# michiyasunaga/qagnn

Hardware: AMD Instinct MI355X
Metric: QA-subgraphs/sec (batch x num_choice) fwd+bwd (higher is better)
Workload: dtype f32; 1 GPU; configs[1]: CSQA-shaped batch 64 questions x 5 choices = 320 subgraphs per GPU, n=200 node slots, 400..2000 edges/subgraph, 38 relations (run_qagnn__csqa.sh), 5-layer GAT d=200 H=4, QAGNN decoder fwd+bwd (LM encoder excluded: random sent_vecs), dropout 0.2, train-mode BN; subgraphs_per_gpu=320, nodes=64000, edges=396800, edges_with_self_loops=460800, graph_input=load-time int32 blobs (qagnn_graph_from_blobs), 13.3 B/edge on the wire, parallelism=single

## Files before the change

qagnn_amd/csrc/gemm_nn2.hip:

```cpp
#include <stdlib.h>

#include <atomic>

#include "common.h"

namespace qagnn {


namespace nn2 {

#ifndef QAGNN_NN2_ABL
#define QAGNN_NN2_ABL 0
#endif

constexpr int BK = 32;
constexpr uint32_t OOB = 0x80000000u;

__device__ __forceinline__ u32x4s bload(__amdgpu_buffer_rsrc_t rsrc, uint32_t voff, uint32_t soff) {
  return __builtin_bit_cast(u32x4s, __builtin_amdgcn_raw_buffer_load_b128(rsrc, (int)voff, (int)soff, 0));
}

__device__ __forceinline__ void split3(uint32_t u, uint32_t& h1, uint32_t& h2, uint32_t& h3) {
  h1 = u & 0xFFFF0000u;
  const float r1 = __builtin_bit_cast(float, u) - __builtin_bit_cast(float, h1);
// ... 365 lines not shown
        }
        QAGNN_NN2_BAR
        QAGNN_NN2_MFMA_TILE3(cur)
        QAGNN_NN2_BAR_VM
      }
      if (g == 0) QAGNN_NN2_BAR
    } else {
    if constexpr (PACKED) {
      QAGNN_NN2_GLDS(0, smem)
    } else {
#pragma unroll
      for (int q = 0; q < BR; ++q) QAGNN_NN2_STORE_B(q, smem)
    }
    QAGNN_NN2_SPLIT_A(0)
    __syncthreads();
    for (int it = 0; it + 1 < nkt; ++it) {
      unsigned char* const cur = smem + (it & 1) * IMG;
      unsigned char* const nxt = smem + ((it & 1) ^ 1) * IMG;
      if constexpr (PACKED && !(QAGNN_NN2_ABL & 2)) QAGNN_NN2_GLDS(it + 1, nxt)
      if constexpr (!(QAGNN_NN2_ABL & 1)) QAGNN_NN2_GLOAD(it + 1)
      QAGNN_NN2_MFMA_TILE(cur, nxt, !PACKED && !(QAGNN_NN2_ABL & 2))
      if constexpr (!(QAGNN_NN2_ABL & 4)) QAGNN_NN2_SPLIT_A(it + 1)
      if constexpr (!(QAGNN_NN2_ABL & 8)) __syncthreads();
    }
    {
      unsigned char* const cur = smem + ((nkt - 1) & 1) * IMG;
      QAGNN_NN2_MFMA_TILE(cur, cur, false)
    }
    }
    if constexpr (NP <= 2) {
      const uint32_t* const bfield = reinterpret_cast<const uint32_t*>(pk + ((int64_t)nkt * ldn1 + 13) * (NP * 1024)) + n0 / 16;
#pragma unroll
      for (int j = 0; j < NT; ++j) {
        const float inv = h2_inv_scale(fa, bfield[j]);
#pragma unroll
        for (int i = 0; i < 2; ++i) acc[i][j] *= inv;
      }
    }
    if constexpr (DIRECT) {
      const int em0 = m0, en0 = n0;
      if constexpr (STAG) {
        loaded = vb + (int)gridDim.x < ntiles;
        if (loaded) {
          QAGNN_NN2_SET_TILE(vb + (int)gridDim.x)
          QAGNN_NN2_FIRST_LOADS
        }
      }
      const __amdgpu_buffer_rsrc_t rC = __builtin_amdgcn_make_buffer_rsrc(a.C, 0, M * a.ldc * 4, 0x00020000);
      const int c4 = 4 * (lane >> 4);
      uint32_t crow[2];
#pragma unroll
      for (int i = 0; i < 2; ++i) {
        const int row = em0 + w * 32 + i * 16 + (lane & 15);
        const bool rok = row < M;
        crow[i] = rok ? (uint32_t)row * (uint32_t)a.ldc * 4u : OOB;
        f32x4s t[NT];
        if (a.bias) {
#pragma unroll
          for (int j = 0; j < NT; ++j) t[j] = __builtin_bit_cast(f32x4s, ld4(a.bias + min(en0 + j * 16 + c4, No - 4)));
#pragma unroll
          for (int j = 0; j < NT; ++j) acc[i][j] += t[j];
        }
        if (a.rowtab) {
          const float* const trow = a.rowtab + (int64_t)a.rowidx[rok ? row : 0] * a.ldt;
#pragma unroll
          for (int j = 0; j < NT; ++j) t[j] = __builtin_bit_cast(f32x4s, ld4(trow + min(en0 + j * 16 + c4, No - 4)));
#pragma unroll
          for (int j = 0; j < NT; ++j) acc[i][j] += t[j];
        }
        if (a.accumulate) {
#pragma unroll
          for (int j = 0; j < NT; ++j) {
            const int col = en0 + j * 16 + c4;
            t[j] = __builtin_bit_cast(f32x4s, bload(rC, rok && col < No ? crow[i] + (uint32_t)col * 4u : OOB, 0u));
          }
#pragma unroll
          for (int j = 0; j < NT; ++j) acc[i][j] += t[j];
        }
      }
#pragma unroll
      for (int i = 0; i < 2; ++i)
#pragma unroll
        for (int j = 0; j < NT; ++j) {
          const int col = en0 + j * 16 + c4;
          const uint32_t off = crow[i] != OOB && col < No ? crow[i] + (uint32_t)col * 4u : OOB;
          if constexpr (QAGNN_NN2_ABL & 64) {
            if (acc[i][j][0] == 1.2345e-30f) __builtin_amdgcn_raw_buffer_store_b128(__builtin_bit_cast(u32x4s, acc[i][j]), rC, (int)off, 0, 0);
          } else {
            __builtin_amdgcn_raw_buffer_store_b128(__builtin_bit_cast(u32x4s, acc[i][j]), rC, (int)off, 0, 0);
          }
        }
      continue;
    }
#undef QAGNN_NN2_FRAG
#undef QAGNN_NN2_FRAG_WAIT
#undef QAGNN_NN2_MFMA_TILE3
#undef QAGNN_NN2_BAR
#undef QAGNN_NN2_BAR_VM
#undef QAGNN_NN2_BAR_VMN
#undef QAGNN_NN2_FIRST_LOADS
#undef QAGNN_NN2_GLOAD
#undef QAGNN_NN2_SET_TILE
#undef QAGNN_NN2_GLDS
#undef QAGNN_NN2_STORE_B
#undef QAGNN_NN2_SPLIT_A
#undef QAGNN_NN2_MFMA_TILE

    float* const St = reinterpret_cast<float*>(smem) + w * SLAB_ROWS * PS;
    float (*const cstat)[2][BN] = reinterpret_cast<float (*)[2][BN]>(smem + SLAB_B);
    constexpr int ROW_F4 = BN / 4, TILE_F4 = SLAB_ROWS * ROW_F4, ST_IT = (TILE_F4 + 63) / 64;
    constexpr int SC = (BN + 63) / 64;
    float x0r[SC], s1[SC], s2v[SC];
#pragma unroll
    for (int cc = 0; cc < SC; ++cc) x0r[cc] = s1[cc] = s2v[cc] = 0.f;
#pragma unroll
    for (int i = 0; i < 2; ++i) {
      __syncthreads();
      const int lr0 = (lane >> 4) * 4;
#pragma unroll
      for (int j = 0; j < NT; ++j)
#pragma unroll
        for (int r = 0; r < 4; ++r) St[(lr0 + r) * PS + j * 16 + (lane & 15)] = acc[i][j][r];
      __syncthreads();
      if constexpr (STATS) {
        const float* const S0 = reinterpret_cast<const float*>(smem) + (w & ~3) * SLAB_ROWS * PS;
#pragma unroll
        for (int cc = 0; cc < SC; ++cc) {
          const int c = lane + cc * 64;
          if (c < BN && n0 + c < No) {
            const float bcv = a.bias ? a.bias[n0 + c] : 0.f;
            if (i == 0) x0r[cc] = S0[c] + bcv;
            const int rows = M - (m0 + (w * 2 + i) * 16);
            float v[SLAB_ROWS];
#pragma unroll
            for (int r = 0; r < SLAB_ROWS; ++r) v[r] = St[r * PS + c];
#pragma unroll
            for (int r = 0; r < SLAB_ROWS; ++r) {
              const float dlt = r < rows ? (v[r] + bcv) - x0r[cc] : 0.f;
              s1[cc] += dlt;
              s2v[cc] = fmaf(dlt, dlt, s2v[cc]);
            }
          }
        }
      }
#pragma unroll
      for (int itx = 0; itx < ST_IT; ++itx) {
        const int idx = lane + itx * 64;
        if (idx >= TILE_F4) break;
        const int slr = idx / ROW_F4, c4 = idx % ROW_F4;
        const int row = m0 + (w * 2 + i) * 16 + slr, col = n0 + c4 * 4;
        if (row >= M || col >= No) continue;
        float4 v = ld4(St + slr * PS + c4 * 4);
        if (a.bias) v = add4(v, ld4(a.bias + col));
        if (a.rowtab) v = add4(v, ld4(a.rowtab + (int64_t)a.rowidx[row] * a.ldt + col));
        float* dst = a.C + (int64_t)row * a.ldc + col;
        if (a.accumulate) v = add4(v, ld4(dst));
        if constexpr (QAGNN_NN2_ABL & 64) {
          if (v.x == 1.2345e-30f) st4(dst, v);
        } else {
          st4(dst, v);
        }
      }
    }
    if constexpr (STATS) {
#pragma unroll
      for (int cc = 0; cc < SC; ++cc) {
        const int c = lane + cc * 64;
        if (c < BN) { cstat[w][0][c] = s1[cc]; cstat[w][1][c] = s2v[cc]; }
      }
      __syncthreads();
      const int hw = w & 3, hf = w >> 2, col = hw * 64 + lane;
      if (col < BN && n0 + col < No && m0 + hf * 128 < M) {
        float x0c = x0r[0];
#pragma unroll
        for (int cc = 1; cc < SC; ++cc) x0c = (hw == cc) ? x0r[cc] : x0c;
        float* const pt = a.colstat_part + ((int64_t)(tile / ncb) * (WV / 4) + hf) * 3 * No + n0 + col;
        const int w0 = hf * 4;
        pt[0] = x0c;
        pt[No] = (cstat[w0][0][col] + cstat[w0 + 1][0][col]) + (cstat[w0 + 2][0][col] + cstat[w0 + 3][0][col]);
        pt[2 * No] = (cstat[w0][1][col] + cstat[w0 + 1][1][col]) + (cstat[w0 + 2][1][col] + cstat[w0 + 3][1][col]);
      }
    }
  }
}
#undef QAGNN_NN2_SIX
#undef QAGNN_NN2_SIX_T

static int num_cus() {
  static int n = [] {
    int dev = 0, v = 0;
    if (hipGetDevice(&dev) != hipSuccess || hipDeviceGetAttribute(&v, hipDeviceAttributeMultiprocessorCount, dev) != hipSuccess || v <= 0) v = 256;
    return v;
  }();
  return n;
}

template <int NT, bool AFFINE, bool STATS, int NP, bool PACKED, int WV>
static int launch_i(const qagnn_gemm_nn_args& b, const float* B1n, int ldn1, const float* B2n, int ldn2, int grid, int ntiles, hipStream_t stream) {
  const size_t lds = nn2_lds_bytes<NT, STATS, WV, NP>(AFFINE ? 2 * ((b.K1 + 31) & ~31) * 4 : 0);
  constexpr int lds_max = nn2_lds_bytes<NT, STATS, WV, NP>(AFFINE ? 2 * 256 * 4 : 0);
  static bool raised[64] = {};
  int dev = 0;
  if (hipGetDevice(&dev) != hipSuccess) dev = 0;
  if (lds_max > 64 * 1024 && !raised[dev & 63]) {
    hipError_t e = hipFuncSetAttribute((const void*)k_gemm_nn2<NT, AFFINE, STATS, NP, PACKED, WV>, hipFuncAttributeMaxDynamicSharedMemorySize, lds_max);
    if (e != hipSuccess) { set_error("gemm_nn2: cannot raise the dynamic LDS limit: %s", hipGetErrorString(e)); return QAGNN_EHIP; }
    raised[dev & 63] = true;
  }
  k_gemm_nn2<NT, AFFINE, STATS, NP, PACKED, WV><<<grid, WV * 64, lds, stream>>>(b, B1n, ldn1, B2n, ldn2, ntiles);
  QAGNN_LAUNCH_CHECK("k_gemm_nn2");
  return QAGNN_OK;
}

template <int NT, int NP, bool PACKED = false, int WV = 4>
static int launch_nt(const qagnn_gemm_nn_args& a, const float* B1n, int ldn1, const float* B2n, int ldn2, hipStream_t stream) {
  qagnn_gemm_nn_args b = a;
  b.xcd_remap = 1;
  const int ntiles = cdiv(a.No, NT * 16) * cdiv(a.M, WV * 32);
  const int cap = (num_cus() * (WV == 8 ? 1 : 2)) & ~7;
  const int grid = ntiles < cap ? ntiles : cap;
  if constexpr (NT == 13 || NT == 7 || NT == 4 || NT == 2) {
    if (a.colstat_part) return launch_i<NT, false, true, NP, PACKED, WV>(b, B1n, ldn1, B2n, ldn2, grid, ntiles, stream);
  }
  if (a.a_scale) return launch_i<NT, true, false, NP, PACKED, WV>(b, B1n, ldn1, B2n, ldn2, grid, ntiles, stream);
  return launch_i<NT, false, false, NP, PACKED, WV>(b, B1n, ldn1, B2n, ldn2, grid, ntiles, stream);
}

template <int NP>
__device__ __forceinline__ void pack_b_wave(const float* __restrict__ B1n, int ldn1, int K1, const float* __restrict__ B2n, int ldn2, int K2, int No,
                                            int NJ, int nkt, int it, int j, unsigned char* __restrict__ out) {
  const int lane = threadIdx.x & 63;
  if (j >= NJ) return;
  float sb = 1.f;
  if constexpr (NP <= 2) {
    const int nn = j * 16 + (lane & 15);
    float m = 0.f;
    if (nn < No) {
      for (int k = (lane >> 4) * 4; k < K1; k += 16) {
        const float4 v = ld4(B1n + (int64_t)nn * ldn1 + k);
        m = fmaxf(fmaxf(m, fmaxf(fabsf(v.x), fabsf(v.y))), fmaxf(fabsf(v.z), fabsf(v.w)));
      }
      for (int k = (lane >> 4) * 4; k < K2; k += 16) {
        const float4 v = ld4(B2n + (int64_t)nn * ldn2 + k);
        m = fmaxf(fmaxf(m, fmaxf(fabsf(v.x), fabsf(v.y))), fmaxf(fabsf(v.z), fabsf(v.w)));
      }
    }
    const uint32_t fb = h2_scale_field(__builtin_bit_cast(uint32_t, wave_max(m)));
    sb = h2_field_to_scale(fb);
    if (it == 0 && lane == 0) reinterpret_cast<uint32_t*>(out + ((int64_t)nkt * NJ + 13) * (NP * 1024))[j] = fb;
  }
  const int r1 = K2 > 0 ? (K1 & 31) : 0;
  const int mixi = r1 != 0 ? 1 : 0;
  const int n1 = mixi ? (K1 >> 5) : ((K1 + 31) >> 5);
  const int s2 = mixi ? 32 - r1 : 0;
  const int kk = (lane >> 4) * 8, n = j * 16 + (lane & 15);
  const float* src = nullptr;
  if (n < No) {
    if (mixi && it == 0) {
      if (kk < r1) src = B1n + (int64_t)n * ldn1 + (K1 - r1 + kk);
      else if (kk - r1 < K2) src = B2n + (int64_t)n * ldn2 + (kk - r1);
    } else {
      const int u = it - mixi;
      if (u < n1) {
        if (u * 32 + kk < K1) src = B1n + (int64_t)n * ldn1 + (u * 32 + kk);
      } else {
        const int k2 = s2 + (u - n1) * 32 + kk;
        if (k2 < K2) src = B2n + (int64_t)n * ldn2 + k2;
      }
    }
  }
  u32x4s r[2] = {{0u, 0u, 0u, 0u}, {0u, 0u, 0u, 0u}};
  if (src) {
    r[0] = *reinterpret_cast<const u32x4s*>(src);
    r[1] = *reinterpret_cast<const u32x4s*>(src + 4);
  }
  u32x4s f[NP];
  if constexpr (NP <= 2) split_frag2<false, NP>(r, f, nullptr, nullptr, 0.f, sb);
  else split_frag<false>(r, f, nullptr, nullptr, 0.f);
  unsigned char* dst = out + ((int64_t)it * NJ + j) * (NP * 1024) + (((lane & 15) ^ (2 * (lane >> 4))) + 16 * (lane >> 4)) * 16;
#pragma unroll
  for (int p = 0; p < NP; ++p) *reinterpret_cast<u32x4s*>(dst + p * 1024) = f[p];
}

template <int NP>
__global__ __launch_bounds__(256) void k_pack_b(const float* __restrict__ B1n, int ldn1, int K1, const float* __restrict__ B2n, int ldn2, int K2,
                                               int No, int NJ, int nkt, unsigned char* __restrict__ out) {
  pack_b_wave<NP>(B1n, ldn1, K1, B2n, ldn2, K2, No, NJ, nkt, blockIdx.y, blockIdx.x * 4 + (threadIdx.x >> 6), out);
}

constexpr int PACK_MAX = 60;
struct PackOne { const float* B1n; const float* B2n; long long out_off; int ldn1, K1, ldn2, K2, No, NJ, jb, blk0, np, nkt; };
struct PackArgs { int n; int nblk; PackOne d[PACK_MAX]; };
__global__ __launch_bounds__(256) void k_pack_b_multi(PackArgs a, unsigned char* __restrict__ out) {
  int i = 0;
  while (i + 1 < a.n && (int)blockIdx.x >= a.d[i + 1].blk0) ++i;
  const PackOne& d = a.d[i];
  const int lb = (int)blockIdx.x - d.blk0;
  const int it = lb / d.jb, j = (lb % d.jb) * 4 + (threadIdx.x >> 6);
  if (d.np == 2) pack_b_wave<2>(d.B1n, d.ldn1, d.K1, d.B2n, d.ldn2, d.K2, d.No, d.NJ, d.nkt, it, j, out + d.out_off);
  else if (d.np == 1) pack_b_wave<1>(d.B1n, d.ldn1, d.K1, d.B2n, d.ldn2, d.K2, d.No, d.NJ, d.nkt, it, j, out + d.out_off);
  else pack_b_wave<3>(d.B1n, d.ldn1, d.K1, d.B2n, d.ldn2, d.K2, d.No, d.NJ, d.nkt, it, j, out + d.out_off);
}

static int walk_tiles(int K1, int K2) {
  const int r1 = K2 > 0 ? (K1 & 31) : 0;
  const int mixi = r1 != 0 ? 1 : 0;
  const int n1 = mixi ? (K1 >> 5) : ((K1 + 31) >> 5);
  const int s2 = mixi ? 32 - r1 : 0;
  const int n2 = K2 > s2 ? ((K2 - s2 + 31) >> 5) : 0;
  return mixi + n1 + n2;
}

}

static std::atomic<int64_t> g_pack_min_m{8192};
int64_t nn2_pack_min_m() { return g_pack_min_m.load(std::memory_order_relaxed); }
bool nn2_packed_ok(const qagnn_gemm_nn_args& a, int64_t ws_bytes, int np) { return a.M >= nn2_pack_min_m() && ws_bytes >= nn2_pack_bytes(a.No, a.K1, a.K2, np); }
static bool nn2_staggered(int nt, const qagnn_gemm_nn_args& a) {
  return nt >= 8 && nn2::walk_tiles(a.K1, a.K2) >= 10 && (int64_t)cdiv(a.No, nt * 16) * cdiv(a.M, 256) * 10 >= nn2::num_cus() * 9;
}
static int launch_nn2_image(int nt, const qagnn_gemm_nn_args& a, const float* p, int NJ, hipStream_t stream, int np = 3) {
  if (np == 1) {
    switch (nt) {
      case 13: return nn2::launch_nt<13, 1, true>(a, p, NJ, nullptr, 0, stream);
      case 8: return nn2::launch_nt<8, 1, true>(a, p, NJ, nullptr, 0, stream);
      case 7: return nn2::launch_nt<7, 1, true>(a, p, NJ, nullptr, 0, stream);
      case 4: return nn2::launch_nt<4, 1, true>(a, p, NJ, nullptr, 0, stream);
      default: return nn2::launch_nt<2, 1, true>(a, p, NJ, nullptr, 0, stream);
    }
  }
  if (np == 2) {
    switch (nt) {
      case 13: return nn2::launch_nt<13, 2, true>(a, p, NJ, nullptr, 0, stream);
      case 8: return nn2::launch_nt<8, 2, true>(a, p, NJ, nullptr, 0, stream);
      case 7: return nn2::launch_nt<7, 2, true>(a, p, NJ, nullptr, 0, stream);
      case 4: return nn2::launch_nt<4, 2, true>(a, p, NJ, nullptr, 0, stream);
      default: return nn2::launch_nt<2, 2, true>(a, p, NJ, nullptr, 0, stream);
    }
  }
  if (nn2_staggered(nt, a)) {
    if (nt == 13) return nn2::launch_nt<13, 3, true, 8>(a, p, NJ, nullptr, 0, stream);
    return nn2::launch_nt<8, 3, true, 8>(a, p, NJ, nullptr, 0, stream);
  }
  switch (nt) {
    case 13: return nn2::launch_nt<13, 3, true>(a, p, NJ, nullptr, 0, stream);
    case 8: return nn2::launch_nt<8, 3, true>(a, p, NJ, nullptr, 0, stream);
    case 7: return nn2::launch_nt<7, 3, true>(a, p, NJ, nullptr, 0, stream);
    case 4: return nn2::launch_nt<4, 3, true>(a, p, NJ, nullptr, 0, stream);
    default: return nn2::launch_nt<2, 3, true>(a, p, NJ, nullptr, 0, stream);
  }
}

bool nn2_ok(const qagnn_gemm_nn_args& a, int ldn1, int ldn2) {
  const int64_t lim = (int64_t)0x7FFFFFFF;
  if (a.a_rowidx && !(a.a_rows > 0 && a.a_rows * (int64_t)a.lda1 * 4 < lim && a.K2 == 0)) return false;
  if (a.K1 % 8 != 0 || a.K2 % 8 != 0) return false;
  if ((int64_t)a.M * a.lda1 * 4 >= lim || (int64_t)a.No * ldn1 * 4 >= lim || (int64_t)a.M * a.ldc * 4 >= lim) return false;
  if (a.K2 > 0 && ((int64_t)a.M * a.lda2 * 4 >= lim || (int64_t)a.No * ldn2 * 4 >= lim)) return false;
  if (a.K2 > 0 && (a.K1 & 31) != 0 && a.K2 < 32 - (a.K1 & 31)) return false;
  if (a.a_scale && a.K1 > 256) return false;
  return true;
}

int launch_nn2(int nt, const qagnn_gemm_nn_args& a, const float* B1n, int ldn1, const float* B2n, int ldn2, hipStream_t stream) {
  switch (nt) {
    case 13: return nn2::launch_nt<13, 3>(a, B1n, ldn1, B2n, ldn2, stream);
    case 8: return nn2::launch_nt<8, 3>(a, B1n, ldn1, B2n, ldn2, stream);
    case 7: return nn2::launch_nt<7, 3>(a, B1n, ldn1, B2n, ldn2, stream);
    case 4: return nn2::launch_nt<4, 3>(a, B1n, ldn1, B2n, ldn2, stream);
    default: return nn2::launch_nt<2, 3>(a, B1n, ldn1, B2n, ldn2, stream);
  }
}

int64_t nn2_pack_bytes(int No, int K1, int K2, int np) {
  const int64_t img = ((int64_t)nn2::walk_tiles(K1, K2) * cdiv(No, 16) + 13) * (np * 1024);
  return np <= 2 ? img + (((int64_t)cdiv(No, 16) + 13) * 4 + 15) / 16 * 16 : img;
}
bool nn2_h2_ok(const qagnn_gemm_nn_args& a) { return a.a_amax1 != nullptr && (a.K2 == 0 || a.a_amax2 != nullptr) && a.M >= nn2_pack_min_m(); }

int launch_nn2_packed(int nt, const qagnn_gemm_nn_args& a, const float* B1n, int ldn1, const float* B2n, int ldn2, void* ws, hipStream_t stream, int np) {
  const int NJ = cdiv(a.No, 16), nkt = nn2::walk_tiles(a.K1, a.K2);
  if (np == 2) nn2::k_pack_b<2><<<dim3(cdiv(NJ, 4), nkt), 256, 0, stream>>>(B1n, ldn1, a.K1, B2n, ldn2, a.K2, a.No, NJ, nkt, reinterpret_cast<unsigned char*>(ws));
  else if (np == 1) nn2::k_pack_b<1><<<dim3(cdiv(NJ, 4), nkt), 256, 0, stream>>>(B1n, ldn1, a.K1, B2n, ldn2, a.K2, a.No, NJ, nkt, reinterpret_cast<unsigned char*>(ws));
  else nn2::k_pack_b<3><<<dim3(cdiv(NJ, 4), nkt), 256, 0, stream>>>(B1n, ldn1, a.K1, B2n, ldn2, a.K2, a.No, NJ, nkt, reinterpret_cast<unsigned char*>(ws));
  QAGNN_LAUNCH_CHECK("k_pack_b");
  return launch_nn2_image(nt, a, reinterpret_cast<const float*>(ws), NJ, stream, np);
}

}
#include <mutex>
#include <vector>
namespace qagnn {
struct PrepackEntry { long long tag; const float* B1n; const float* B2n; int ldn1, K1, ldn2, K2, No, np; const void* pk; };
static std::mutex g_prepack_mu;
static std::vector<PrepackEntry> g_prepack;

const void* nn2_prepack_lookup(const float* B1n, int ldn1, int K1, const float* B2n, int ldn2, int K2, int No, int np) {
  std::lock_guard<std::mutex> lk(g_prepack_mu);
  for (size_t i = g_prepack.size(); i-- > 0;) {
    const PrepackEntry& e = g_prepack[i];
    if (e.np == np && e.B1n == B1n && e.K1 == K1 && e.No == No && e.ldn1 == ldn1 && e.K2 == K2 && (K2 == 0 || (e.B2n == B2n && e.ldn2 == ldn2))) return e.pk;
  }
  return nullptr;
}

static bool prepack_takes(const qagnn_pack_desc& d) {
  if (!d.B1n || d.No <= 0 || d.K1 < 8 || d.K1 % 8 != 0 || d.K2 < 0 || d.K2 % 8 != 0 || d.ldn1 < d.K1 || d.ldn1 % 4 != 0 || !aligned16(d.B1n)) return false;
  if (d.K2 > 0 && (!d.B2n || d.ldn2 < d.K2 || d.ldn2 % 4 != 0 || !aligned16(d.B2n))) return false;
  if (d.K2 > 0 && (d.K1 & 31) != 0 && d.K2 < 32 - (d.K1 & 31)) return false;
  return true;
}

int launch_nn2_prepacked(int nt, const qagnn_gemm_nn_args& a, const void* pk, hipStream_t stream, int np) {
  return launch_nn2_image(nt, a, reinterpret_cast<const float*>(pk), cdiv(a.No, 16), stream, np);
}
}

using namespace qagnn;

extern "C" int64_t qagnn_packed_min_rows(int64_t rows) {
  return rows < 0 ? g_pack_min_m.load() : g_pack_min_m.exchange(rows > 1 ? rows : 1);
}

extern "C" int64_t qagnn_gemm_nn_prepack_bytes(const qagnn_pack_desc* d, int32_t n) {
  int64_t tot = 0;
  for (int i = 0; i < n; ++i)
    if (prepack_takes(d[i])) tot += nn2_pack_bytes(d[i].No, d[i].K1, d[i].K2, (d[i].pieces == 2 || d[i].pieces == 1) ? d[i].pieces : 3);
  return tot;
}

extern "C" int qagnn_gemm_nn_prepack_clear(int64_t tag) {
  std::lock_guard<std::mutex> lk(g_prepack_mu);
  size_t keep = 0;
  for (size_t i = 0; i < g_prepack.size(); ++i)
    if (!(tag == 0 || g_prepack[i].tag == tag)) g_prepack[keep++] = g_prepack[i];
  g_prepack.resize(keep);
  return QAGNN_OK;
}

extern "C" int qagnn_gemm_nn_prepack_f32(const qagnn_pack_desc* d, int32_t n, void* out, int64_t out_bytes, int64_t tag, qagnn_stream_t stream_) {
  QAGNN_REQUIRE(d && n > 0 && out && tag != 0 && aligned16(out), QAGNN_EINVAL, "gemm_nn_prepack: bad arguments");
  QAGNN_REQUIRE(out_bytes >= qagnn_gemm_nn_prepack_bytes(d, n), QAGNN_EINVAL, "gemm_nn_prepack: the buffer of %lld bytes is too small", (long long)out_bytes);
  qagnn_gemm_nn_prepack_clear(tag);
  std::vector<PrepackEntry> fresh;
  int64_t off = 0;
  for (int i0 = 0; i0 < n;) {
    nn2::PackArgs pa;
    pa.n = 0;
    pa.nblk = 0;
    int i = i0;
    for (; i < n && pa.n < nn2::PACK_MAX; ++i) {
      if (!prepack_takes(d[i])) continue;
      nn2::PackOne& o = pa.d[pa.n++];
      o.B1n = d[i].B1n; o.B2n = d[i].K2 > 0 ? d[i].B2n : nullptr; o.ldn1 = d[i].ldn1; o.K1 = d[i].K1; o.ldn2 = d[i].ldn2; o.K2 = d[i].K2; o.No = d[i].No;
      o.NJ = cdiv(d[i].No, 16);
      o.jb = cdiv(o.NJ, 4);
      o.blk0 = pa.nblk;
      o.out_off = off;
      o.np = (d[i].pieces == 2 || d[i].pieces == 1) ? d[i].pieces : 3;
      o.nkt = nn2::walk_tiles(o.K1, o.K2);
      pa.nblk += o.jb * o.nkt;
      fresh.push_back(PrepackEntry{(long long)tag, o.B1n, o.B2n, o.ldn1, o.K1, o.ldn2, o.K2, o.No, o.np, static_cast<const unsigned char*>(out) + off});
      off += nn2_pack_bytes(o.No, o.K1, o.K2, o.np);
    }
    if (pa.n > 0) {
      nn2::k_pack_b_multi<<<pa.nblk, 256, 0, (hipStream_t)stream_>>>(pa, static_cast<unsigned char*>(out));
      QAGNN_LAUNCH_CHECK("k_pack_b_multi");
    }
    i0 = i;
  }
  std::lock_guard<std::mutex> lk(g_prepack_mu);
  g_prepack.insert(g_prepack.end(), fresh.begin(), fresh.end());
  return QAGNN_OK;
}
```

Baseline: 44150 QA-subgraphs/s.

## Add LDS-resident packed-B GEMM kernel with persistent row-task loop

Adds a persistent GEMM variant that loads an entire column slab of the prepacked fp16-split weight image into LDS (up to 160 KB) once per block, then streams 32-row A tiles through it with 16 waves per block distributed per XCD. It is selected by default for 1- or 2-piece packed GEMMs whose slab fits, avoiding repeated B-image reloads per output tile. The tradeoffs are large LDS use, which limits each CU to one block, and a fixed 7-column-tile width. Shapes that need column statistics or have large K still take the old path.

Result: slower. 42140 QA-subgraphs/s, median of 2 (-4.5%).

```diff
diff --git a/qagnn_amd/csrc/gemm_nn2.hip b/qagnn_amd/csrc/gemm_nn2.hip
--- a/qagnn_amd/csrc/gemm_nn2.hip
+++ b/qagnn_amd/csrc/gemm_nn2.hip
@@ -691,7 +691,7 @@
   else pack_b_wave<3>(d.B1n, d.ldn1, d.K1, d.B2n, d.ldn2, d.K2, d.No, d.NJ, d.nkt, it, j, out + d.out_off);
 }
 
-static int walk_tiles(int K1, int K2) {
+constexpr int walk_tiles(int K1, int K2) {
   const int r1 = K2 > 0 ? (K1 & 31) : 0;
   const int mixi = r1 != 0 ? 1 : 0;
   const int n1 = mixi ? (K1 >> 5) : ((K1 + 31) >> 5);
@@ -700,6 +700,278 @@
   return mixi + n1 + n2;
 }
 
+constexpr int RES_NT = 7;
+constexpr int RES_WV = 16;
+constexpr int RES_LDS_LIMIT = 160 * 1024;
+constexpr int64_t res_slab_bytes(int K1, int K2, int No, int np, bool affine) {
+  if (np < 1 || np > 2 || K1 < 8 || No < 1) return 0;
+  if ((No + 15) / 16 < RES_NT) return 0;
+  const int64_t b = (int64_t)walk_tiles(K1, K2) * RES_NT * np * 1024 + (affine ? 2 * ((K1 + 31) & ~31) * 4 : 0);
+  return b <= RES_LDS_LIMIT ? b : 0;
+}
+static_assert(res_slab_bytes(208, 0, 208, 2, true) == 98 * 1024 + 2 * 224 * 4, "208 -> 208: 7 k-tiles x 7 column tiles x 2 pieces + scale / shift");
+static_assert(res_slab_bytes(208, 112, 624, 2, false) == 140 * 1024, "[208 | 112] -> 624: 10 k-tiles x 7 column tiles x 2 pieces");
+static_assert(res_slab_bytes(624, 0, 208, 2, false) == 0 && res_slab_bytes(624, 0, 112, 2, false) == 0, "K = 624 (20 k-tiles, 280 KB) does not fit");
+
+template <int NT, bool AFFINE, int NP, int WV>
+__global__ __launch_bounds__(WV * 64) __attribute__((amdgpu_waves_per_eu(WV / 4, WV / 4))) void k_gemm_nn2r(qagnn_gemm_nn_args a,
+                                                                                                   const unsigned char* __restrict__ pk,
+                                                                                                   int NJ, int nslab, int rg) {
+  static_assert(NP == 1 || NP == 2, "the scaled fp16 forms");
+  constexpr int IMG = NT * NP * 1024;
+  extern __shared__ __attribute__((aligned(16))) unsigned char smem[];
+
+  const int tid = threadIdx.x, lane = tid & 63;
+  const int w = __builtin_amdgcn_readfirstlane(tid >> 6);
+  const int M = a.M, No = a.No, K1 = a.K1, K2 = a.K2;
+  const int r1 = K2 > 0 ? (K1 & 31) : 0;
+  const int mixi = r1 != 0 ? 1 : 0;
+  const int n1 = mixi ? (K1 >> 5) : ((K1 + 31) >> 5);
+  const int s2 = mixi ? 32 - r1 : 0;
+  const int n2 = K2 > s2 ? ((K2 - s2 + 31) >> 5) : 0;
+  const int nkt = mixi + n1 + n2;
+  const int KA = (K1 + 31) & ~31;
+  float* const aff = reinterpret_cast<float*>(smem + nkt * IMG);
+
+  const int xcd = (int)blockIdx.x & 7, slot = (int)blockIdx.x >> 3;
+  const int slab = slot % nslab, g = slot / nslab;
+  const int ntask = (M + 31) >> 5;
+  const int tq = ntask >> 3, tr = ntask & 7;
+  const int t0 = xcd < tr ? xcd * (tq + 1) : tr * (tq + 1) + (xcd - tr) * tq;
+  const int t1 = t0 + tq + (xcd < tr ? 1 : 0);
+  const int stride = rg * WV;
+  if (g >= rg || t0 + g * WV >= t1) return;
+  int task = t0 + g * WV + w;
+  const int n0 = slab * NT * 16;
+
+  const __amdgpu_buffer_rsrc_t rA1 = __builtin_amdgcn_make_buffer_rsrc(const_cast<float*>(a.A1), 0, (a.a_rowidx ? (int)a.a_rows : M) * a.lda1 * 4, 0x00020000);
+  const __amdgpu_buffer_rsrc_t rA2 = __builtin_amdgcn_make_buffer_rsrc(const_cast<float*>(a.A2), 0, K2 > 0 ? M * a.lda2 * 4 : 0, 0x00020000);
+  const __amdgpu_buffer_rsrc_t rC = __builtin_amdgcn_make_buffer_rsrc(a.C, 0, M * a.ldc * 4, 0x00020000);
+
+  {
+    const unsigned char* const src = pk + (int64_t)(n0 / 16) * (NP * 1024) + lane * 16;
+    const int nb = nkt * NT * NP;
+    for (int b = w; b < nb; b += WV) {
+      const int it = b / (NT * NP), r = b - it * (NT * NP);
+      __builtin_amdgcn_global_load_lds((const __attribute__((address_space(1))) void*)(src + ((int64_t)it * NJ * NP + r) * 1024),
+                                       (__attribute__((address_space(3))) void*)(smem + b * 1024), 16, 0, 0);
+    }
+  }
+  if constexpr (AFFINE) {
+    for (int i = tid; i < 2 * KA; i += WV * 64) {
+      const int k = i < KA ? i : i - KA;
+      aff[i] = k < K1 ? (i < KA ? a.a_scale[k] : a.a_shift[k]) : 0.f;
+    }
+  }
+  uint32_t fa = 127u;
+  float sa = 1.f;
+  {
+    uint32_t mb = a.a_amax1[0];
+    if (K2 > 0 && a.a_amax2) mb = max(mb, a.a_amax2[0]);
+    fa = __builtin_amdgcn_readfirstlane(h2_scale_field(mb));
+    sa = h2_field_to_scale(fa);
+  }
+  const int ac = lane >> 4;
+  const int rd_off = (((lane & 15) ^ (2 * ac)) + 16 * ac) * 16;
+  const int c4i = 4 * (lane >> 4);
+
+  uint32_t arow1[2], arow2[2];
+  u32x4s ra[2][2];
+  auto set_rows = [&](int t) {
+#pragma unroll
+    for (int i = 0; i < 2; ++i) {
+      const int row = t * 32 + i * 16 + (lane & 15);
+      const int64_t grow = (a.a_rowidx && row < M) ? a.a_rowidx[row] : (int64_t)row;
+      arow1[i] = (row < M && grow >= 0) ? (uint32_t)grow * (uint32_t)a.lda1 * 4u + (uint32_t)ac * 32u : OOB;
+      arow2[i] = row < M ? (uint32_t)row * (uint32_t)a.lda2 * 4u + (uint32_t)ac * 32u : OOB;
+    }
+  };
+  auto gload = [&](int it) {
+    const int u = it - mixi;
+    if (u < n1) {
+      const int kb = u * 32;
+      const bool ain = kb + ac * 8 < K1;
+#pragma unroll
+      for (int i = 0; i < 2; ++i) {
+        const uint32_t off = ain ? arow1[i] : OOB;
+        ra[i][0] = bload(rA1, off, (uint32_t)kb * 4u);
+        ra[i][1] = bload(rA1, off, (uint32_t)kb * 4u + 16u);
+      }
+    } else {
+      const int kb = s2 + (u - n1) * 32;
+      const bool ain = kb + ac * 8 < K2;
+#pragma unroll
+      for (int i = 0; i < 2; ++i) {
+        const uint32_t off = ain ? arow2[i] : OOB;
+        ra[i][0] = bload(rA2, off, (uint32_t)kb * 4u);
+        ra[i][1] = bload(rA2, off, (uint32_t)kb * 4u + 16u);
+      }
+    }
+  };
+  auto first_loads = [&](int t) {
+    if (mixi) {
+      const int kaq = ac * 8;
+      const bool a1 = kaq < r1;
+#pragma unroll
+      for (int i = 0; i < 2; ++i) {
+        const int64_t row = min(t * 32 + i * 16 + (lane & 15), M - 1);
+        const float* p = a1 ? a.A1 + row * a.lda1 + (K1 - r1 + kaq) : a.A2 + row * a.lda2 + (kaq - r1);
+        ra[i][0] = *reinterpret_cast<const u32x4s*>(p);
+        ra[i][1] = *reinterpret_cast<const u32x4s*>(p + 4);
+      }
+    } else {
+      gload(0);
+    }
+  };
+
+  const bool have = task < t1;
+  if (have) {
+    set_rows(task);
+    first_loads(task);
+  }
+  __syncthreads();
+  if (!have) return;
+
+  uint32_t fb[NT];
+  {
+    const uint32_t* const bfield = reinterpret_cast<const uint32_t*>(pk + ((int64_t)nkt * NJ + 13) * (NP * 1024)) + n0 / 16;
+#pragma unroll
+    for (int j = 0; j < NT; ++j) fb[j] = __builtin_amdgcn_readfirstlane(bfield[j]);
+  }
+  while (true) {
+    const int em0 = task * 32;
+    f32x4s acc[2][NT];
+#pragma unroll
+    for (int i = 0; i < 2; ++i)
+#pragma unroll
+      for (int j = 0; j < NT; ++j) acc[i][j] = (f32x4s){0.f, 0.f, 0.f, 0.f};
+
+    for (int it = 0; it < nkt; ++it) {
+      u32x4s af[2][NP];
+      if constexpr (AFFINE) {
+        const int u_ = it - mixi;
+        const bool mixt_ = mixi && it == 0;
+        const bool s1_ = mixt_ ? (ac * 8 < r1) : (u_ < n1);
+        const int k_ = min(mixt_ ? K1 - r1 + ac * 8 : u_ * 32 + ac * 8, KA - 8);
+        const float4 c0 = ld4(aff + k_), c1 = ld4(aff + k_ + 4), h0 = ld4(aff + KA + k_), h1 = ld4(aff + KA + k_ + 4);
+        const float sc[8] = {s1_ ? c0.x : 1.f, s1_ ? c0.y : 1.f, s1_ ? c0.z : 1.f, s1_ ? c0.w : 1.f,
+                             s1_ ? c1.x : 1.f, s1_ ? c1.y : 1.f, s1_ ? c1.z : 1.f, s1_ ? c1.w : 1.f};
+        const float sh[8] = {s1_ ? h0.x : 0.f, s1_ ? h0.y : 0.f, s1_ ? h0.z : 0.f, s1_ ? h0.w : 0.f,
+                             s1_ ? h1.x : 0.f, s1_ ? h1.y : 0.f, s1_ ? h1.z : 0.f, s1_ ? h1.w : 0.f};
+        const float lo = s1_ ? 0.f : -INFINITY;
+#pragma unroll
+        for (int i = 0; i < 2; ++i) split_frag2<true, NP>(ra[i], af[i], sc, sh, lo, sa);
+      } else {
+#pragma unroll
+        for (int i = 0; i < 2; ++i) split_frag2<false, NP>(ra[i], af[i], nullptr, nullptr, 0.f, sa);
+      }
+      if constexpr (!(QAGNN_NN2_ABL & 1)) {
+        if (it + 1 < nkt) gload(it + 1);
+      }
+      const unsigned char* const cur = smem + it * IMG + rd_off;
+      __builtin_amdgcn_s_setprio(1);
+      u32x4s bfa[NP], bfb[NP];
+#pragma unroll
+      for (int p = 0; p < NP; ++p) bfa[p] = *reinterpret_cast<const u32x4s*>(cur + p * 1024);
+#pragma unroll
+      for (int j = 0; j < NT; ++j) {
+        u32x4s(&bf)[NP] = (j & 1) ? bfb : bfa;
+        u32x4s(&bn)[NP] = (j & 1) ? bfa : bfb;
+        if (j + 1 < NT) {
+#pragma unroll
+          for (int p = 0; p < NP; ++p) bn[p] = *reinterpret_cast<const u32x4s*>(cur + ((j + 1) * NP + p) * 1024);
+        }
+        if constexpr (!(QAGNN_NN2_ABL & 32)) {
+#pragma unroll
+          for (int i = 0; i < 2; ++i) acc[i][j] = mfma_pieces<NP, true>(af[i], bf, acc[i][j]);
+        } else {
+#pragma unroll
+          for (int p = 0; p < NP; ++p) asm volatile("" ::"v"(bf[p]), "v"(af[0][p]), "v"(af[1][p]));
+        }
+        __builtin_amdgcn_sched_barrier(0);
+      }
+      __builtin_amdgcn_s_setprio(0);
+    }
+    uint32_t fal = fa;
+    asm volatile("" : "+s"(fal));
+#pragma unroll
+    for (int j = 0; j < NT; ++j) {
+      const float inv = h2_inv_scale(fal, fb[j]);
+#pragma unroll
+      for (int i = 0; i < 2; ++i) acc[i][j] *= inv;
+    }
+    const int next = task + stride;
+    const bool more = next < t1;
+    if (more) {
+      set_rows(next);
+      first_loads(next);
+    }
+    int c4 = c4i;
+    asm volatile("" : "+v"(c4));
+    uint32_t crow[2];
+#pragma unroll
+    for (int i = 0; i < 2; ++i) {
+      const int row = em0 + i * 16 + (lane & 15);
+      const bool rok = row < M;
+      crow[i] = rok ? (uint32_t)row * (uint32_t)a.ldc * 4u : OOB;
+      f32x4s t[NT];
+      if (a.bias) {
+#pragma unroll
+        for (int j = 0; j < NT; ++j) t[j] = __builtin_bit_cast(f32x4s, ld4(a.bias + min(n0 + j * 16 + c4, No - 4)));
+#pragma unroll
+        for (int j = 0; j < NT; ++j) acc[i][j] += t[j];
+      }
+      if (a.rowtab) {
+        const float* const trow = a.rowtab + (int64_t)a.rowidx[rok ? row : 0] * a.ldt;
+#pragma unroll
+        for (int j = 0; j < NT; ++j) t[j] = __builtin_bit_cast(f32x4s, ld4(trow + min(n0 + j * 16 + c4, No - 4)));
+#pragma unroll
+        for (int j = 0; j < NT; ++j) acc[i][j] += t[j];
+      }
+      if (a.accumulate) {
+#pragma unroll
+        for (int j = 0; j < NT; ++j) {
+          const int col = n0 + j * 16 + c4;
+          t[j] = __builtin_bit_cast(f32x4s, bload(rC, rok && col < No ? crow[i] + (uint32_t)col * 4u : OOB, 0u));
+        }
+#pragma unroll
+        for (int j = 0; j < NT; ++j) acc[i][j] += t[j];
+      }
+    }
+#pragma unroll
+    for (int i = 0; i < 2; ++i)
+#pragma unroll
+      for (int j = 0; j < NT; ++j) {
+        const int col = n0 + j * 16 + c4;
+        const uint32_t off = crow[i] != OOB && col < No ? crow[i] + (uint32_t)col * 4u : OOB;
+        if constexpr (QAGNN_NN2_ABL & 64) {
+          if (acc[i][j][0] == 1.2345e-30f) __builtin_amdgcn_raw_buffer_store_b128(__builtin_bit_cast(u32x4s, acc[i][j]), rC, (int)off, 0, 0);
+        } else {
+          __builtin_amdgcn_raw_buffer_store_b128(__builtin_bit_cast(u32x4s, acc[i][j]), rC, (int)off, 0, 0);
+        }
+      }
+    if (!more) break;
+    task = next;
+  }
+}
+
+template <int NT, bool AFFINE, int NP, int WV>
+static int launch_res_i(const qagnn_gemm_nn_args& a, const unsigned char* pk, int NJ, hipStream_t stream) {
+  const int64_t lds = res_slab_bytes(a.K1, a.K2, a.No, NP, AFFINE);
+  static bool raised[64] = {};
+  int dev = 0;
+  if (hipGetDevice(&dev) != hipSuccess) dev = 0;
+  if (!raised[dev & 63]) {
+    hipError_t e = hipFuncSetAttribute((const void*)k_gemm_nn2r<NT, AFFINE, NP, WV>, hipFuncAttributeMaxDynamicSharedMemorySize, RES_LDS_LIMIT);
+    if (e != hipSuccess) { set_error("gemm_nn2r: cannot raise the dynamic LDS limit: %s", hipGetErrorString(e)); return QAGNN_EHIP; }
+    raised[dev & 63] = true;
+  }
+  const int per_xcd = num_cus() / 8, nslab = cdiv(NJ, NT);
+  k_gemm_nn2r<NT, AFFINE, NP, WV><<<per_xcd * 8, WV * 64, (size_t)lds, stream>>>(a, pk, NJ, nslab, per_xcd / nslab);
+  QAGNN_LAUNCH_CHECK("k_gemm_nn2r");
+  return QAGNN_OK;
+}
+
 }
 
 static std::atomic<int64_t> g_pack_min_m{8192};
@@ -708,7 +980,27 @@
 static bool nn2_staggered(int nt, const qagnn_gemm_nn_args& a) {
   return nt >= 8 && nn2::walk_tiles(a.K1, a.K2) >= 10 && (int64_t)cdiv(a.No, nt * 16) * cdiv(a.M, 256) * 10 >= nn2::num_cus() * 9;
 }
+static bool nn2_resident_enabled() {
+  static const int v = getenv("QAGNN_NN_RESIDENT") ? atoi(getenv("QAGNN_NN_RESIDENT")) : 1;
+  return v != 0;
+}
+static bool nn2_resident_ok(const qagnn_gemm_nn_args& a, int np) {
+  if (!nn2_resident_enabled() || np > 2 || a.colstat_part || a.M < nn2_pack_min_m()) return false;
+  if (nn2::res_slab_bytes(a.K1, a.K2, a.No, np, a.a_scale != nullptr) == 0) return false;
+  return cdiv(cdiv(a.No, 16), nn2::RES_NT) <= nn2::num_cus() / 8;
+}
+static int launch_nn2_resident(const qagnn_gemm_nn_args& a, const float* p, int NJ, hipStream_t stream, int np) {
+  const unsigned char* const pk = reinterpret_cast<const unsigned char*>(p);
+  if (np == 1) {
+    return a.a_scale ? nn2::launch_res_i<nn2::RES_NT, true, 1, nn2::RES_WV>(a, pk, NJ, stream)
+                     : nn2::launch_res_i<nn2::RES_NT, false, 1, nn2::RES_WV>(a, pk, NJ, stream);
+  }
+  return a.a_scale ? nn2::launch_res_i<nn2::RES_NT, true, 2, nn2::RES_WV>(a, pk, NJ, stream)
+                   : nn2::launch_res_i<nn2::RES_NT, false, 2, nn2::RES_WV>(a, pk, NJ, stream);
+}
+
 static int launch_nn2_image(int nt, const qagnn_gemm_nn_args& a, const float* p, int NJ, hipStream_t stream, int np = 3) {
+  if (nn2_resident_ok(a, np)) return launch_nn2_resident(a, p, NJ, stream, np);
   if (np == 1) {
     switch (nt) {
       case 13: return nn2::launch_nt<13, 1, true>(a, p, NJ, nullptr, 0, stream);
@@ -806,6 +1098,15 @@
 }
 
 using namespace qagnn;
+
+extern "C" int64_t qagnn_nn_resident_lds_bytes(int32_t M, int32_t K1, int32_t K2, int32_t No, int32_t np, int32_t affine, int32_t stats) {
+  qagnn_gemm_nn_args a = {};
+  static float dummy[4];
+  a.M = M; a.K1 = K1; a.K2 = K2; a.No = No;
+  if (affine) a.a_scale = dummy;
+  if (stats) a.colstat_part = dummy;
+  return nn2_resident_ok(a, np) ? nn2::res_slab_bytes(K1, K2, No, np, affine != 0) : 0;
+}
 
 extern "C" int64_t qagnn_packed_min_rows(int64_t rows) {
   return rows < 0 ? g_pack_min_m.load() : g_pack_min_m.exchange(rows > 1 ? rows : 1);
```
